# mathjeff/Mapper

Hardware: AMD Instinct MI355X
Metric: M reads/s aligned (150 bp) (higher is better)
Workload: dtype f64

## Files before the change

mapper_amd/csrc/xm_defs.h:

```cpp
#pragma once
#include <stdint.h>
#include <stddef.h>
#include <math.h>
#include <stdlib.h>

#if defined(__HIPCC__)
#include <hip/hip_runtime.h>
#define XM_HD __host__ __device__
#if defined(__HIP_DEVICE_COMPILE__)
#define XM_GLOBAL(T) T __attribute__((address_space(1)))
#define XM_LDS(T) T __attribute__((address_space(3)))
#else
#define XM_GLOBAL(T) T
#define XM_LDS(T) T
#endif
#define XM_INL __host__ __device__ __forceinline__
#ifndef XM_NOINL_LINKAGE
#define XM_NOINL_LINKAGE
#endif
#define XM_NOINL XM_NOINL_LINKAGE __host__ __device__ __noinline__
#define XM_NOINL_DECL XM_NOINL_LINKAGE __host__ __device__
#else
#define XM_HD
#define XM_GLOBAL(T) T
#define XM_LDS(T) T
#define XM_INL inline
#define XM_NOINL
#define XM_NOINL_DECL
#endif

namespace xm {

enum : int32_t {
  XM_OK = 0,
  XM_ST_OVERFLOW = 1,
  XM_ST_OUT_OVERFLOW = 2,
  XM_ST_NEED_GROW = 4,
  XM_ST_INTERNAL = 5,
  XM_ST_NEED_HEAVY = 6,
  XM_ST_NEED_CONF = 11,
};

XM_INL int32_t jadd(int32_t a, int32_t b) { return (int32_t)((uint32_t)a + (uint32_t)b); }
XM_INL int32_t jmul(int32_t a, int32_t b) { return (int32_t)((uint32_t)a * (uint32_t)b); }
XM_INL int32_t jabs(int32_t v) { return v == INT32_MIN ? v : (v < 0 ? -v : v); }
XM_INL int32_t j2i(double d) {
  if (d != d) return 0;
  if (d >= 2147483647.0) return INT32_MAX;
  if (d <= -2147483648.0) return INT32_MIN;
  return (int32_t)d;
}
XM_INL double dmin(double a, double b) { return a < b ? a : b; }
XM_INL double dmax(double a, double b) { return a > b ? a : b; }
XM_INL double jmaxd(double a, double b) {
  if (a != a || b != b) return NAN;
  return a > b ? a : b;
}
XM_INL int imin(int a, int b) { return a < b ? a : b; }
XM_INL int iclamp(int v, int lo, int hi) { return v < lo ? lo : (v > hi ? hi : v); }
XM_INL int imax(int a, int b) { return a > b ? a : b; }
XM_INL int iabs(int a) { return a < 0 ? -a : a; }
XM_INL double jnextUp(double d) {
  if (d != d || d == INFINITY) return d;
  if (d == 0.0) { uint64_t b = 1; double r; __builtin_memcpy(&r, &b, 8); return r; }
  uint64_t b;
  __builtin_memcpy(&b, &d, 8);
  if (d > 0) b += 1; else b -= 1;
  double r;
  __builtin_memcpy(&r, &b, 8);
  return r;
}

XM_INL uint8_t bpComplement(uint8_t b) { return (uint8_t)(((b & 1) << 3) | ((b & 2) << 1) | ((b & 4) >> 1) | ((b & 8) >> 3)); }
XM_INL bool bpCanMatch(uint8_t a, uint8_t b) { return (a & b) != 0; }
XM_INL int bpPop(uint8_t b) { return __builtin_popcount(b & 15); }
XM_INL bool bpIsAmbiguous(uint8_t b) { return bpPop(b) != 1; }
XM_INL bool bpIsFullyAmbiguous(uint8_t b) { return (b & 15) == 15; }
XM_INL double bpFalseNegativeRate(uint8_t b) { int n = bpPop(b); return n <= 1 ? 0.0 : (double)(n - 1) / 3.0; }

struct SeqView {
  const uint8_t* base;
  int32_t len;
  uint8_t rc;
  uint8_t id;
  XM_INL uint8_t at(int i) const { XM_GLOBAL(const uint8_t)* const g = (XM_GLOBAL(const uint8_t)*)base; return rc ? bpComplement(g[len - 1 - i]) : g[i]; }
};

XM_INL uint64_t seqWord8(const SeqView& s, int i) {
  uint64_t x;
  if (!s.rc) {
    __builtin_memcpy(&x, (const void*)(s.base + i), 8);
    return x;
  }
  __builtin_memcpy(&x, (const void*)(s.base + (s.len - 8 - i)), 8);
  x = __builtin_bswap64(x);
  return ((x & 0x0101010101010101ull) << 3) | ((x & 0x0202020202020202ull) << 1) | ((x & 0x0404040404040404ull) >> 1) | ((x & 0x0808080808080808ull) >> 3);
}
XM_INL int seqMatchRun(const SeqView& a, int ai, const SeqView& b, int bi, int limit) {
  int k = 0;
  while (k + 8 <= limit && ai + k + 8 <= a.len && bi + k + 8 <= b.len) {
    const uint64_t t = seqWord8(a, ai + k) & seqWord8(b, bi + k);
    const uint64_t zero = ~(t + 0x7F7F7F7F7F7F7F7Full) & 0x8080808080808080ull;
    if (zero) return k + (__builtin_ctzll(zero) >> 3);
    k += 8;
  }
  while (k < limit && bpCanMatch(a.at(ai + k), b.at(bi + k))) k++;
  return k;
}
XM_INL int seqMatchRunBack(const SeqView& a, int ai, const SeqView& b, int bi, int limit) {
  int k = 0;
  while (k + 8 <= limit && ai - k - 7 >= 0 && bi - k - 7 >= 0) {
    const uint64_t t = seqWord8(a, ai - k - 7) & seqWord8(b, bi - k - 7);
    const uint64_t zero = ~(t + 0x7F7F7F7F7F7F7F7Full) & 0x8080808080808080ull;
    if (zero) return k + (__builtin_clzll(zero) >> 3);
    k += 8;
  }
  while (k < limit && bpCanMatch(a.at(ai - k), b.at(bi - k))) k++;
  return k;
}

XM_INL uint64_t seqAmbiguousBytes(uint64_t x) {
  x &= 0x0F0F0F0F0F0F0F0Full;
  const uint64_t pairs = (x & 0x0505050505050505ull) + ((x >> 1) & 0x0505050505050505ull);
  const uint64_t pop = (pairs & 0x0303030303030303ull) + ((pairs >> 2) & 0x0303030303030303ull);
  const uint64_t bad = pop ^ 0x0101010101010101ull;
  return (bad + 0x7F7F7F7F7F7F7F7Full) & 0x8080808080808080ull;
}
XM_INL uint64_t seqZeroBytes(uint64_t t) { return ~(t + 0x7F7F7F7F7F7F7F7Full) & 0x8080808080808080ull; }
XM_INL int seqCountAmbiguous(const SeqView& s, int start, int end) {
  int n = 0, i = start;
  for (; i + 8 <= end && i + 8 <= s.len && i >= 0; i += 8) n += __builtin_popcountll(seqAmbiguousBytes(seqWord8(s, i)));
  for (; i < end; i++) if (__builtin_popcount(s.at(i) & 15) != 1) n++;
  return n;
}

struct Params {
  double MutationPenalty, InsertionStart_Penalty, InsertionExtension_Penalty, DeletionStart_Penalty, DeletionExtension_Penalty,
      MaxErrorRate, UnalignedPenalty, AmbiguityPenalty, Max_PenaltySpan;
  int32_t MaxNumMatches;
  int32_t StartingInsertionStartFree;
  XM_INL double getStartingInsertionStartPenalty() const { return StartingInsertionStartFree ? 0.0 : InsertionStart_Penalty; }
  XM_INL double getMinPossibleNonzeroPenalty() const {
    double r = MutationPenalty;
    r = dmin(r, getStartingInsertionStartPenalty() + InsertionStart_Penalty);
    r = dmin(r, DeletionStart_Penalty + DeletionExtension_Penalty);
    return r;
  }
  XM_INL double getPenalty(uint8_t q, uint8_t r) const {
    if (!bpCanMatch(r, q)) return MutationPenalty;
    return AmbiguityPenalty * bpFalseNegativeRate((uint8_t)(q | r));
  }
};

struct Table {
  int32_t capacity;
  int32_t maxCount;
  int64_t offBase;
  int64_t posBase;
};
static const uint32_t XM_OVERFULL = 0x80000000u;

struct IndexView {
  int32_t numContigs, minInterestingSize, maxHashedLength, enableGapmers, posIs64;
  int32_t dupWindow;
  double dupGranularity;
  int64_t totalForwardAndReverseSize;
  const int64_t* contigStart;
  const int32_t* contigLen;
  const int64_t* seqCumStart;
  const uint8_t* refCodes;
  const Table* tables;
  const uint32_t* bucketOff;
  const uint32_t* positions32;
  const uint64_t* positions64;
  const int64_t* dupKeyStart;
  const int32_t* dupKeys;
  const uint32_t* lines32;
  const uint64_t* lines64;
  const struct ConfEntry* conf;
  uint32_t confMask;
  struct ConfMiss* confMiss;
  const int32_t* baLogStep;
};
struct ConfEntry { uint64_t penaltyBits; int32_t queryLength; int32_t used; double totalLengthForHighConfidence; };
struct ConfMissKey { uint64_t penaltyBits; int32_t queryLength; int32_t pad; };
struct ConfMiss { unsigned long long n; unsigned long long cap; ConfMissKey keys[1]; };
XM_INL uint32_t confHash(uint64_t penaltyBits, int32_t queryLength) {
  uint64_t x = (penaltyBits ^ (penaltyBits >> 31)) * 0x9E3779B97F4A7C15ull + (uint64_t)(uint32_t)queryLength * 0xC2B2AE3D27D4EB4Full;
  return (uint32_t)(x >> 37);
}
XM_INL bool confLookup(const ConfEntry* table, uint32_t mask, double penalty, int32_t queryLength, double& value) {
  if (!table) return false;
  uint64_t bits;
  __builtin_memcpy(&bits, &penalty, 8);
  uint32_t h = confHash(bits, queryLength) & mask;
  while (true) {
    const ConfEntry e = table[h];
    if (!e.used) return false;
    if (e.penaltyBits == bits && e.queryLength == queryLength) { value = e.totalLengthForHighConfidence; return true; }
    h = (h + 1) & mask;
  }
}
XM_INL int32_t baNumBasesToEncodeReferencePosition(const int32_t* step, int32_t refLen) {
  if (refLen == 0) return INT32_MIN + 1;
  if (refLen < 0) return 1;
  int k = 0;
  while (k + 1 < 24 && refLen >= step[k + 1]) k++;
  return k + 1;
}
constexpr int XM_LINE_SLOTS = 7;
constexpr int64_t XM_LINE_FLAG = 1ll << 62;
template <typename W, typename P>
XM_INL void xmFillLine(W* line, uint32_t o0, uint32_t o1, const P* tablePositions) {
  const uint32_t first = o0 & ~XM_OVERFULL, count = (o1 & ~XM_OVERFULL) - first;
  line[0] = (W)(count | (o0 & XM_OVERFULL));
  for (uint32_t j = 0; j < (uint32_t)XM_LINE_SLOTS; j++) line[1 + j] = ((o0 & XM_OVERFULL) == 0 && j < count) ? (W)tablePositions[first + j] : (W)0;
}

XM_INL SeqView refView(const IndexView& ix, int contig, bool rc) {
  SeqView v;
  v.base = ix.refCodes + ix.contigStart[contig];
  v.len = ix.contigLen[contig];
  v.rc = rc ? 1 : 0;
  v.id = 0;
  return v;
}

struct Caps {
  int32_t scale;
  int32_t heavyAllowed;
  int32_t searchInHbmOnly;
  int32_t maxLevels, maxPyramidBlocks, maxHistory, maxCounters, maxPending, maxQM, maxGoodAlignments, maxBlocks,
      maxNodes, nodeHash, gridCap, maxBuckets, bucketHash, matcherEntries, maxSections, maxPieces, maxCountMap, maxJoined;
};
XM_INL Caps makeCaps(int scale) {
  Caps c;
  c.scale = scale;
  c.heavyAllowed = 2;
  c.searchInHbmOnly = 0;
  c.maxLevels = 48 * scale;
  c.maxPyramidBlocks = 1536 * scale;
  c.maxHistory = 192 * scale;
  c.maxCounters = 96 * scale;
  c.maxPending = 128 * scale;
  c.maxQM = 64 * scale;
  c.maxGoodAlignments = 32 * scale;
  c.maxBlocks = 16 * scale;
  c.maxNodes = 1536 * scale;
  c.nodeHash = 4096 * scale;
// ... 57 lines not shown
```

mapper_amd/csrc/xm_seed.h:

```cpp
#pragma once
#include "xm_defs.h"

#ifndef XM_WALK_INLINE
#define XM_WALK_INLINE 2
#endif
#if XM_WALK_INLINE >= 1
#define XM_NOINL_W1 XM_INL
#else
#define XM_NOINL_W1 XM_NOINL
#endif
#if XM_WALK_INLINE >= 2
#define XM_NOINL_W2 XM_INL
#else
#define XM_NOINL_W2 XM_NOINL
#endif
#if XM_WALK_INLINE == 3
#define XM_NOINL_W3 XM_INL
#else
#define XM_NOINL_W3 XM_NOINL
#endif
#if XM_WALK_INLINE >= 4
#define XM_NOINL_W4 XM_INL
#else
#define XM_NOINL_W4 XM_NOINL
#endif

namespace xm {

struct alignas(16) PBlock {
  uint16_t start, len;
  int32_t fwd, rev;
  uint8_t flags;
  int8_t gapDir;
  int16_t extraGap;
};
enum : uint8_t { F_RML = 1, F_RMR = 2, F_NRML = 4, F_NRMR = 8 };
struct alignas(16) PBlockWord { uint32_t w[4]; };
XM_INL PBlock pbUnpack(const PBlockWord& v) {
  PBlock b;
  b.start = (uint16_t)(v.w[0] & 0xFFFFu); b.len = (uint16_t)(v.w[0] >> 16); b.fwd = (int32_t)v.w[1]; b.rev = (int32_t)v.w[2];
  b.flags = (uint8_t)(v.w[3] & 0xFFu); b.gapDir = (int8_t)((v.w[3] >> 8) & 0xFFu); b.extraGap = (int16_t)(v.w[3] >> 16);
  return b;
}
XM_INL PBlockWord pbPack(const PBlock& b) {
  PBlockWord v;
  v.w[0] = (uint32_t)b.start | ((uint32_t)b.len << 16); v.w[1] = (uint32_t)b.fwd; v.w[2] = (uint32_t)b.rev;
  v.w[3] = (uint32_t)b.flags | ((uint32_t)(uint8_t)b.gapDir << 8) | ((uint32_t)(uint16_t)b.extraGap << 16);
  return v;
}

XM_INL int maxGapmerNumBasepairsUsed(int startingLength) { return startingLength + startingLength * 9 / 8 + 1; }

XM_INL PBlock level0Block(uint8_t code, int index) {
  PBlock b;
  int f = (code == 1) ? 0 : (code == 2) ? 1 : (code == 4) ? 2 : 3;
  b.start = (uint16_t)index;
  b.len = 1;
  b.fwd = f;
  b.rev = 3 - f;
  b.flags = (uint8_t)(((f / 2 == 0) ? F_RML : F_RMR) | ((f % 2 == 0) ? F_NRML : F_NRMR));
  b.gapDir = 0;
  b.extraGap = 0;
  return b;
}

XM_INL int32_t mergeHash(int leftLength, int32_t leftHash, int rightLength, int32_t rightHash) {
  int64_t rotatedLeft = ((int64_t)leftHash + 1) * (54323 + 323 * (int64_t)rightLength);
  int64_t rotatedRight = (int64_t)jadd(rightHash, 1) * (int64_t)leftLength;
  uint64_t top = (uint64_t)rotatedLeft + (uint64_t)rotatedRight;
  return jadd((int32_t)(uint32_t)top, (int32_t)(uint32_t)((uint64_t)((int64_t)top >> 32)));
}

template <typename B>
XM_INL bool shouldMergeBlocks(const B& l, const B& r) {
  if ((int)l.start + l.len < (int)r.start) return false;
  return (l.flags & F_RMR) || (r.flags & F_RML);
}

constexpr uint8_t mergeRule(int anchor, int fr, int aBits, int oBits, int lc) {
  bool rml = true, rmr = true, nrml = true, nrmr = true;
  if (anchor != 0 && fr != 1) {
    bool anchorIsRight = anchor == 2;
    bool isReverse = fr == 0;
    bool invert = isReverse == anchorIsRight;
    bool aL = (aBits & 1) != 0, aR = (aBits & 2) != 0;
    if (aL && aR) { if (anchorIsRight) aR = false; else aL = false; }
    bool oL = (oBits & 1) != 0, oR = (oBits & 2) != 0;
    if (oL && oR) { if (!anchorIsRight) oL = false; else oR = false; }
    rml = aL != invert;
    rmr = aR != invert;
    nrml = oL != invert;
    nrmr = oR != invert;
  }
  if (lc != 1) {
    rml = lc == 2;
    rmr = !rml;
    nrml = !rml;
    nrmr = !nrml;
  }
  if (fr != 1) {
    if (rml && rmr) { rml = fr == 2; rmr = !rml; }
    if (nrml && nrmr) { nrml = rml; nrmr = !nrml; }
  }
  int gd = 0;
  if (rml != rmr) gd = rml ? 1 : -1;
  else if (anchor != 0) gd = (anchor == 2) ? 1 : -1;
  return (uint8_t)((rml ? F_RML : 0) | (rmr ? F_RMR : 0) | (nrml ? F_NRML : 0) | (nrmr ? F_NRMR : 0) | ((gd + 1) << 4));
}
struct MergeRuleTable { uint8_t v[3 * 3 * 4 * 4 * 3]; };
constexpr MergeRuleTable makeMergeRuleTable() {
  MergeRuleTable t{};
  for (int anchor = 0; anchor < 3; anchor++) for (int fr = 0; fr < 3; fr++) for (int a = 0; a < 4; a++) for (int o = 0; o < 4; o++) for (int lc = 0; lc < 3; lc++)
    t.v[(((anchor * 3 + fr) * 4 + a) * 4 + o) * 3 + lc] = mergeRule(anchor, fr, a, o, lc);
  return t;
}
static constexpr MergeRuleTable kMergeRuleHost = makeMergeRuleTable();
#if defined(__HIPCC__)
static __device__ const MergeRuleTable kMergeRuleDev = makeMergeRuleTable();
#endif
#if defined(__HIP_DEVICE_COMPILE__)
__shared__ uint8_t xm_merge_rule_lds[sizeof(MergeRuleTable)];
XM_INL void xmLoadMergeRule() {
  for (int i = (int)threadIdx.x; i < (int)sizeof(MergeRuleTable); i += (int)blockDim.x) xm_merge_rule_lds[i] = kMergeRuleDev.v[i];
  __syncthreads();
}
XM_INL uint8_t mergeRuleLookup(int idx) { return xm_merge_rule_lds[idx]; }
#else
XM_INL void xmLoadMergeRule() {}
XM_INL uint8_t mergeRuleLookup(int idx) { return kMergeRuleHost.v[idx]; }
#endif

template <typename B>
XM_INL B mergeBlocks(const B& L, const B& R) {
  B b;
  int start = L.start, len = (int)R.start + R.len - (int)L.start;
  b.start = (decltype(b.start))start;
  b.len = (decltype(b.len))len;
  b.fwd = mergeHash(L.len, L.fwd, R.len, R.fwd);
  b.rev = mergeHash(R.len, R.rev, L.len, L.rev);
  const int anchor = (L.fwd != R.rev) ? ((L.fwd > R.rev) ? 2 : 1) : 0;
  const int fr = (b.fwd < b.rev) ? 0 : ((b.fwd == b.rev) ? 1 : 2);
  const int lc = (L.len < R.len) ? 0 : ((L.len == R.len) ? 1 : 2);
  const int lBits = (L.flags >> 2) & 3, rBits = (R.flags >> 2) & 3;
  const int aBits = (anchor == 2) ? rBits : lBits, oBits = (anchor == 2) ? lBits : rBits;
  const uint8_t rule = mergeRuleLookup((((anchor * 3 + fr) * 4 + aBits) * 4 + oBits) * 3 + lc);
  b.flags = (uint8_t)(rule & 15);
  b.gapDir = (int8_t)((int)(rule >> 4) - 1);
  b.extraGap = (int16_t)(((int)L.len + (int)R.len - len) / 4);
  return b;
}

struct QBlock {
  int32_t start, len, used, fwd, rev;
  int32_t id;
  uint8_t flags;
  XM_INL int end() const { return start + len; }
  XM_INL bool isPrimaryPolarity() const {
    bool rml = (flags & F_RML) != 0, rmr = (flags & F_RMR) != 0;
    if (rml != rmr) return rml;
    return fwd >= rev;
  }
  XM_INL int32_t lookupKey() const { return isPrimaryPolarity() ? fwd : rev; }
};

XM_INL int gapmerCharCode(uint8_t code) {
  return code == 1 ? 1 : code == 2 ? 2 : code == 4 ? 3 : code == 8 ? 4 : 0;
}

template <typename B>
XM_INL int withGapAndExtension(const B& b, const SeqView& seq, QBlock& out) {
  int targetExtraLength = b.len;
  int32_t mx = b.fwd > b.rev ? b.fwd : b.rev;
  targetExtraLength += jabs(mx) % 3;
  targetExtraLength += b.extraGap;
  int gapLength = b.len / 2;
  int extensionLength = targetExtraLength - gapLength;
  out.flags = 0;
// ... 81 lines not shown
  int32_t* status;
  DevCounters* dc;

  XM_INL void init(const SeqView& s, PBlock* b, int cap_, int32_t* ls, int maxLevels_, int32_t* st) {
    dc = nullptr;
    ms = nullptr;
    seq = s; blocks = b; cap = cap_; levelStart = ls; maxLevels = maxLevels_; nBuilt = 0; used = 0; status = st;
    levelStart[1] = 0;
  }

  XM_INL PBlock entryAt(int level, int i) const {
    if (level > 0) return blocks[levelStart[level] + i];
    uint8_t code = seq.at(i);
    PBlock b = level0Block(code, i);
    if (bpIsAmbiguous(code)) { b.flags = F_MULTI; b.fwd = 0; b.rev = 0; }
    return b;
  }
  XM_INL int numPoss(int level, const PBlock& e) const {
    if (!(e.flags & F_MULTI)) return 1;
    if (level > 0) return e.rev;
    return bpPop(seq.at(e.start));
  }
  XM_INL void possAt(int level, const PBlock& e, int k, PossView& p) const {
    if (!(e.flags & F_MULTI)) { p.block = e; p.cond = &p.own; p.condLen = 0; p.hasBlock = 1; return; }
    if (level > 0) {
      const Poss& s = ms->pool[e.fwd + k];
      p.block = s.block; p.cond = ms->conds + s.condOff; p.condLen = s.condLen; p.hasBlock = s.hasBlock;
      return;
    }
    uint8_t code = seq.at(e.start);
    int seen = 0;
    uint8_t option = 1;
    for (int bit = 0; bit < 4; bit++) {
      uint8_t o = (uint8_t)(1 << bit);
      if (code & o) { if (seen == k) { option = o; break; } seen++; }
    }
    p.block = level0Block(option, e.start);
    p.own = ((CondEnt)e.start << 2) | (CondEnt)(option == 1 ? 0 : option == 2 ? 1 : option == 4 ? 2 : 3);
    p.cond = &p.own; p.condLen = 1;
    p.hasBlock = 1;
  }
  XM_INL bool multiAddOption(int& nOpt, int& nOptCond, const PBlock& block, bool hasBlock, const CondEnt* cond, int condLen) {
    if (ms->poolUsed + nOpt >= ms->poolCap || ms->condUsed + nOptCond + condLen > ms->condCap) return false;
    Poss& o = ms->pool[ms->poolUsed + nOpt];
    o.block = block; o.hasBlock = hasBlock ? 1 : 0; o.pad = 0;
    o.condOff = ms->condUsed + nOptCond; o.condLen = condLen;
    for (int t = 0; t < condLen; t++) ms->conds[o.condOff + t] = cond[t];
    nOpt++; nOptCond += condLen;
    return true;
  }
  XM_INL bool multiExpand(int prev, int n, const PBlock& leftBlock, const CondEnt* leftCond, int leftCondLen, int i, int& nOpt, int& nOptCond) {
    MFrame* const st = ms->frames;
    CondEnt* const sc = ms->stack;
    if (leftCondLen > ms->stackCap || ms->framesCap < 1) return false;
    for (int t = 0; t < leftCondLen; t++) sc[t] = leftCond[t];
    int sp = 0;
    st[0].j = i; st[0].opt = 0; st[0].condOff = 0; st[0].condLen = leftCondLen; st[0].found = 0;
    while (sp >= 0) {
      MFrame& f = st[sp];
      const int nextIdx = f.j + 1;
      if (nextIdx >= n) { sp--; continue; }
      const PBlock next = entryAt(prev, nextIdx);
      if (f.opt >= numPoss(prev, next)) { sp--; continue; }
      PossView ro;
      possAt(prev, next, f.opt, ro);
      f.opt++;
      const int top = f.condOff + f.condLen;
      const int icLen = condIntersect(sc + f.condOff, f.condLen, ro.cond, ro.condLen, sc + top, ms->stackCap - top);
      if (icLen == -2) return false;
      if (icLen < 0) { if (f.found) sp--; continue; }
      f.found = 1;
      if (nOpt > XM_MAX_COMBINATIONS) return true;
      if (!ro.hasBlock) {
        if (sp + 1 >= ms->framesCap) return false;
        sp++;
        st[sp].j = nextIdx; st[sp].opt = 0; st[sp].condOff = top; st[sp].condLen = icLen; st[sp].found = 0;
        continue;
      }
      const bool merge = shouldMergeBlocks(leftBlock, ro.block);
      if (!multiAddOption(nOpt, nOptCond, merge ? mergeBlocks(leftBlock, ro.block) : leftBlock, merge, sc + top, icLen)) return false;
    }
    return true;
  }
  XM_INL void buildLevelMulti() {
    const int prev = nBuilt;
    const int n = count(prev);
    int w = used;
    for (int i = 0; i + 1 < n; i++) {
      const PBlock L = entryAt(prev, i), R = entryAt(prev, i + 1);
      if (!((L.flags | R.flags) & F_MULTI)) {
        if (shouldMergeBlocks(L, R)) {
          if (w >= cap) { *status = XM_ST_OVERFLOW; return; }
          blocks[w++] = mergeBlocks(L, R);
        }
        continue;
      }
      int nOpt = 0, nOptCond = 0;
      const int nl = numPoss(prev, L);
      for (int k = 0; k < nl; k++) {
        PossView lo;
        possAt(prev, L, k, lo);
        if (lo.hasBlock) {
          if (!multiExpand(prev, n, lo.block, lo.cond, lo.condLen, i, nOpt, nOptCond)) { *status = XM_ST_OVERFLOW; return; }
        } else {
          if (!multiAddOption(nOpt, nOptCond, lo.block, false, lo.cond, lo.condLen)) { *status = XM_ST_OVERFLOW; return; }
        }
      }
      if (nOpt > 0 && nOpt <= XM_MAX_COMBINATIONS) {
        int minStart = -1, maxEnd = -1;
        for (int k = 0; k < nOpt; k++) if (ms->pool[ms->poolUsed + k].hasBlock) {
          const PBlock& b = ms->pool[ms->poolUsed + k].block;
          if (minStart < 0 || (int)b.start < minStart) minStart = b.start;
          if ((int)b.start + b.len > maxEnd) maxEnd = (int)b.start + b.len;
        }
        if (minStart >= 0) {
          if (w >= cap) { *status = XM_ST_OVERFLOW; return; }
          PBlock m;
          m.start = (uint16_t)minStart; m.len = (uint16_t)(maxEnd - minStart); m.fwd = ms->poolUsed; m.rev = nOpt; m.flags = F_MULTI; m.gapDir = 0; m.extraGap = 0;
          ms->poolUsed += nOpt; ms->condUsed += nOptCond;
          blocks[w++] = m;
        }
      }
    }
    nBuilt++;
    used = w;
    levelStart[nBuilt + 1] = w;
  }
  XM_INL int count(int level) const { return level == 0 ? seq.len : levelStart[level + 1] - levelStart[level]; }
  XM_INL PBlock blockAt(int level, int i) const { return level == 0 ? level0Block(seq.at(i), i) : blocks[levelStart[level] + i]; }

  XM_NOINL void ensureMulti(int level) {
    while (nBuilt < level) {
      if (nBuilt + 2 >= maxLevels) { *status = XM_ST_OVERFLOW; return; }
      buildLevelMulti();
      if (*status) return;
    }
  }
  XM_NOINL void ensure(int level) {
    if (ms) { ensureMulti(level); return; }
    XM_TIC(t0);
    PBlock* const blk = blocks;
    const int capL = cap;
    const SeqView sq = seq;
    while (nBuilt < level) {
      if (nBuilt + 2 >= maxLevels) { *status = XM_ST_OVERFLOW; return; }
      int prev = nBuilt;
      int n = count(prev);
      int w = used;
      const int base = prev == 0 ? 0 : levelStart[prev];
      bool ovf = false;
      if (n > 1 && prev == 0) {
        XM_GLOBAL(PBlockWord)* const dst = (XM_GLOBAL(PBlockWord)*)blk;
        PBlock L = level0Block(sq.at(0), 0);
        for (int i0 = 0; i0 + 1 < n && !ovf; i0 += 8) {
          uint8_t codes[8];
          const int m = imin(8, n - 1 - i0);
#pragma unroll
          for (int k = 0; k < 8; k++) codes[k] = sq.at(i0 + 1 + (k < m ? k : 0));
#pragma unroll
          for (int k = 0; k < 8; k++) {
            if (k < m && !ovf) {
              const PBlock R = level0Block(codes[k], i0 + 1 + k);
              if (shouldMergeBlocks(L, R)) {
                if (w >= capL) ovf = true;
                else dst[w++] = pbPack(mergeBlocks(L, R));
              }
              L = R;
            }
          }
        }
      } else if (n > 1) {
        XM_GLOBAL(const PBlockWord)* const src = (XM_GLOBAL(const PBlockWord)*)(blk + base);
        XM_GLOBAL(PBlockWord)* const dst = (XM_GLOBAL(PBlockWord)*)blk;
        PBlock L = pbUnpack(src[0]);
        for (int i0 = 0; i0 + 1 < n && !ovf; i0 += 8) {
          PBlockWord buf[8];
          const int m = imin(8, n - 1 - i0);
#pragma unroll
          for (int k = 0; k < 8; k++) buf[k] = src[i0 + 1 + (k < m ? k : 0)];
#pragma unroll
          for (int k = 0; k < 8; k++) {
            if (k < m && !ovf) {
              const PBlock R = pbUnpack(buf[k]);
              if (shouldMergeBlocks(L, R)) {
                if (w >= capL) ovf = true;
                else dst[w++] = pbPack(mergeBlocks(L, R));
              }
              L = R;
            }
          }
        }
      }
      if (ovf) { *status = XM_ST_OVERFLOW; return; }
      nBuilt++;
      used = w;
      levelStart[nBuilt + 1] = w;
    }
    XM_TOC(dc, T_PYRAMID, t0);
  }
  XM_INL bool getAfter(int level, int pos, PBlock& out) {
    if (level == 0) {
      int p = pos + 1;
      if (p >= seq.len) return false;
      out = ms ? entryAt(0, p) : level0Block(seq.at(p), p);
      return true;
    }
    ensure(level);
    if (*status) return false;
    int lo = levelStart[level], hi = levelStart[level + 1];
    while (lo < hi) {
      int mid = (lo + hi) >> 1;
      if ((int)blocks[mid].start > pos) hi = mid; else lo = mid + 1;
    }
    if (lo >= levelStart[level + 1]) return false;
    out = blocks[lo];
    return true;
  }
  XM_INL bool get(int level, int index, PBlock& out) {
    if (level == 0) {
      if (index >= seq.len) return false;
      out = ms ? entryAt(0, index) : level0Block(seq.at(index), index);
      return true;
    }
    if (!getAfter(level, index - 1, out)) return false;
    return (int)out.start == index;
  }
};

XM_INL const Table* containingMap(const IndexView& ix, int used, int32_t* status) {
  if (used > ix.maxHashedLength) { *status = XM_ST_NEED_GROW; return nullptr; }
  return &ix.tables[used];
}
XM_INL uint32_t packedKey(const Table* t, int32_t key) {
  int32_t r = key % t->capacity;
  if (r < 0) r += t->capacity;
  return (uint32_t)r;
}
XM_INL int numMatchesLowerBound(const IndexView& ix, const QBlock& b, DevCounters* dc, int32_t* status) {
  if (b.used < ix.minInterestingSize) return INT32_MAX;
  const Table* t = containingMap(ix, b.used, status);
  if (!t) return INT32_MAX;
  uint32_t k = packedKey(t, b.lookupKey());
  if (dc) dc->headerProbes++;
  if (ix.lines32 || ix.lines64) {
    const uint32_t h = ix.lines64 ? (uint32_t)ix.lines64[(t->offBase + k) * 8] : ix.lines32[(t->offBase + k) * 8];
    return (h & XM_OVERFULL) ? INT32_MAX : (int)h;
  }
  const uint32_t* off = ix.bucketOff + t->offBase + k;
  uint32_t o0 = off[0], o1 = off[1];
  if (o0 & XM_OVERFULL) return INT32_MAX;
  return (int)((o1 & ~XM_OVERFULL) - (o0 & ~XM_OVERFULL));
}
XM_INL int dbMaxNumMatchesAllowed(const IndexView& ix, const QBlock& b, int32_t* status) {
  if (b.used < ix.minInterestingSize) return -1;
  const Table* t = containingMap(ix, b.used, status);
  if (!t) return 0;
  return t->maxCount;
}
struct RefPos { int32_t contig; uint8_t rc; int32_t start; };
XM_INL RefPos decodePosition(const IndexView& ix, int64_t enc) {
  int lo = 0, hi = ix.numContigs * 2;
  while (hi - lo > 1) {
    int mid = (lo + hi) >> 1;
    if (ix.seqCumStart[mid] <= enc) lo = mid; else hi = mid;
  }
  RefPos p;
  p.contig = lo >> 1;
  p.rc = (uint8_t)(lo & 1);
  p.start = (int32_t)(enc - ix.seqCumStart[lo]);
  return p;
}
XM_INL int64_t xmPositionAt(const IndexView& ix, int64_t idx) {
  if (idx & XM_LINE_FLAG) { idx &= ~XM_LINE_FLAG; return ix.lines64 ? (int64_t)ix.lines64[idx] : (int64_t)ix.lines32[idx]; }
  return ix.posIs64 ? (int64_t)ix.positions64[idx] : (int64_t)ix.positions32[idx];
}
XM_INL int matchBlock(const IndexView& ix, const QBlock& b, int64_t& first, bool& invert, DevCounters* dc, int32_t* status) {
  if (b.used < ix.minInterestingSize) return -1;
  const Table* t = containingMap(ix, b.used, status);
  if (!t) return -1;
  uint32_t k = packedKey(t, b.lookupKey());
  if (dc) { dc->headerProbes++; dc->bucketFetches++; }
  int count;
  if (ix.lines32 || ix.lines64) {
    const int64_t line = (t->offBase + k) * 8;
    const uint32_t h = ix.lines64 ? (uint32_t)ix.lines64[line] : ix.lines32[line];
    if (h & XM_OVERFULL) return -1;
    count = (int)h;
    if (count > t->maxCount) return -1;
    if (count <= XM_LINE_SLOTS) first = XM_LINE_FLAG | (line + 1);
    else first = t->posBase + (int64_t)(ix.bucketOff[t->offBase + k] & ~XM_OVERFULL);
  } else {
    const uint32_t* off = ix.bucketOff + t->offBase + k;
    uint32_t o0 = off[0], o1 = off[1];
    if (o0 & XM_OVERFULL) return -1;
    count = (int)((o1 & ~XM_OVERFULL) - (o0 & ~XM_OVERFULL));
    if (count > t->maxCount) return -1;
    first = t->posBase + (int64_t)(o0 & ~XM_OVERFULL);
  }
  invert = !b.isPrimaryPolarity();
  if (dc) dc->hitsFetched += (unsigned long long)count;
  return count;
}
XM_INL RefPos fetchHit(const IndexView& ix, int64_t idx, bool invert, int blockSpan) {
  int64_t enc = xmPositionAt(ix, idx);
  RefPos p = decodePosition(ix, enc);
  if (invert) {
    p.start = ix.contigLen[p.contig] - p.start - blockSpan;
    p.rc ^= 1;
  }
  return p;
}

struct PathState {
  int32_t batchIndex;
  bool curExists;
  PBlock cur;
  bool gapComputed;
  int32_t gapStatus;
  QBlock gap;
  bool havePrev1, havePrev2;
  int32_t prevFwd1, prevFwd2;
};

struct Counter {
  int32_t offset;
  int32_t contig;
  int32_t numMatches, numDistinctMismatches, lastMismatchedPosition, lastMatchedBlockId, historyProcessedIndex, priority;
  int32_t next, prev;
  uint8_t seqAId;
  uint8_t mapSel;
  uint8_t good;
};

struct SeqMatch {
  int32_t offset, contig;
  uint8_t seqAId;
  XM_INL bool reversed() const { return (seqAId & 1) != 0; }
};

struct QMatch {
  int32_t n, priority;
  SeqMatch c[2];
  uint8_t hint;
};

struct ListRef { int32_t id, n; int16_t* items; };

struct ReadCtx;

struct Comp {
  Pyramid pyr;
  PathState path;
  SeqView query, rcQuery;
  Counter* counters; int32_t nCounters;
  int16_t* good; int32_t nGood;
  bool foundGood, done;
  QBlock* history; int32_t nHistory;
  QBlock* pending; int32_t pendHead, pendTail;
  int32_t numBlocksMatchingAnywhere, maxNonoverlappingBlockVisited, numNonoverlappingBlocksVisited, minNumDistinctMismatches;
  int32_t maxIndelLengthToConsider;
  int32_t nextBlockId;
  ListRef hp, best, all;
};

struct SeedEnv {
  const IndexView* ix;
  const Caps* caps;
  DevCounters* dc;
  int32_t* status;
  int32_t* listIdCounter;
  const int32_t* mateLen;
};

XM_INL int seqALen(const SeedEnv& e, uint8_t seqAId) { return e.mateLen[seqAId >> 1]; }
XM_INL int smStartB(const SeqMatch& m) { return imax(0, m.offset); }
XM_INL int smEndB(const SeedEnv& e, const SeqMatch& m) { return imin(m.offset + seqALen(e, m.seqAId), e.ix->contigLen[m.contig]); }
XM_INL bool smEquals(const SeqMatch& a, const SeqMatch& b) { return a.offset == b.offset && a.seqAId == b.seqAId && a.contig == b.contig; }

XM_INL void pathInit(PathState& p) {
  p.batchIndex = -1;
  p.curExists = true;
  p.cur.start = 0; p.cur.len = 0; p.cur.fwd = 0; p.cur.rev = 0; p.cur.flags = 0; p.cur.gapDir = 0; p.cur.extraGap = 0;
  p.gapComputed = false;
  p.gapStatus = 0;
  p.havePrev1 = p.havePrev2 = false;
  p.prevFwd1 = p.prevFwd2 = 0;
}

XM_INL void pathMoveRight(Comp& c) {
  PBlock nb;
  c.path.curExists = c.pyr.getAfter(c.path.batchIndex, c.path.cur.start, nb);
  if (c.path.curExists) c.path.cur = nb;
  c.path.gapComputed = false;
}
XM_INL void pathMoveDown(Comp& c) {
  c.path.batchIndex--;
  PBlock nb;
  c.path.curExists = c.pyr.getAfter(c.path.batchIndex, c.path.cur.start, nb);
  if (c.path.curExists) c.path.cur = nb;
  c.path.gapComputed = false;
}
XM_INL void pathMoveUpOrRight(Comp& c) {
  PBlock up;
  if (c.pyr.get(c.path.batchIndex + 1, c.path.cur.start, up)) {
    c.path.batchIndex++;
    c.path.cur = up;
    c.path.gapComputed = false;
  } else {
    pathMoveRight(c);
  }
}
XM_INL bool pathWithGap(Comp& c, const SeedEnv& e, QBlock& out) {
  if (!e.ix->enableGapmers) {
    const PBlock& b = c.path.cur;
    out.start = b.start; out.len = b.len; out.used = b.len; out.fwd = b.fwd; out.rev = b.rev; out.flags = b.flags; out.id = -1;
    return true;
  }
  if (!c.path.gapComputed) {
    c.path.gapStatus = withGapAndExtension(c.path.cur, c.pyr.seq, c.path.gap);
    c.path.gap.id = -1;
    c.path.gapComputed = true;
  }
  if (c.path.gapStatus == 0) return false;
  out = c.path.gap;
  return true;
}
XM_INL int pathMaxNumMatchesAllowed(Comp& c, const SeedEnv& e, const QBlock& b) {
  if (b.len >= c.query.len / 6) return dbMaxNumMatchesAllowed(*e.ix, b, e.status);
  if (b.flags & F_RMR) return 5;
  return b.used + 1;
}
XM_NOINL_W1 bool pathAdvance(Comp& c, const SeedEnv& e) {
  XM_TIC(t0);
  int singleLen = c.path.cur.len;
  if (maxGapmerNumBasepairsUsed(singleLen) < e.ix->minInterestingSize && e.ix->enableGapmers) {
    pathMoveUpOrRight(c);
  } else {
    QBlock ext;
    if (pathWithGap(c, e, ext)) {
      int numMatches = numMatchesLowerBound(*e.ix, ext, e.dc, e.status);
      if (numMatches < 6) {
        if (c.path.batchIndex > 0) pathMoveDown(c); else pathMoveRight(c);
      } else {
        if (numMatches > pathMaxNumMatchesAllowed(c, e, ext)) pathMoveUpOrRight(c);
        else pathMoveRight(c);
      }
    } else {
      int typical = singleLen * 3 / 2;
      if (typical <= e.ix->minInterestingSize && e.ix->enableGapmers) pathMoveUpOrRight(c);
      else { if (c.path.batchIndex > 0) pathMoveDown(c); else pathMoveRight(c); }
    }
  }
  while (c.path.curExists && (c.path.cur.flags & F_MULTI) && *e.status == 0) {
    if (c.path.batchIndex > 0) pathMoveDown(c); else pathMoveRight(c);
  }
  XM_TOC(e.dc, T_WALK, t0);
  return c.path.curExists && *e.status == 0;
}
XM_NOINL_W1 bool pathNextInterestingBlock(Comp& c, const SeedEnv& e, QBlock& out) {
  if (!c.path.curExists) return false;
  while (true) {
    if (!pathAdvance(c, e)) return false;
    QBlock ext;
    if (!pathWithGap(c, e, ext)) continue;
    int n = numMatchesLowerBound(*e.ix, ext, e.dc, e.status);
    if (*e.status) return false;
    if (!(n <= pathMaxNumMatchesAllowed(c, e, ext))) continue;
    bool seen = false;
    if (c.path.havePrev1 && ext.fwd == c.path.prevFwd1) seen = true;
    else if (c.path.havePrev2 && ext.fwd == c.path.prevFwd2) seen = true;
    c.path.havePrev2 = c.path.havePrev1;
    c.path.prevFwd2 = c.path.prevFwd1;
    c.path.havePrev1 = true;
    c.path.prevFwd1 = ext.fwd;
    if (seen) continue;
    ext.id = c.nextBlockId++;
    out = ext;
    return true;
  }
}

XM_INL void counterUpdate(Comp& c, const SeedEnv& e, Counter& k) {
  while (k.historyProcessedIndex < c.nHistory) {
    const QBlock& b = c.history[k.historyProcessedIndex];
    if (b.id != k.lastMatchedBlockId) {
      if (b.start >= k.lastMismatchedPosition) {
        if (k.offset + b.end() <= e.ix->contigLen[k.contig]) {
          k.numDistinctMismatches++;
          k.lastMismatchedPosition = b.end();
        }
      }
    }
    k.historyProcessedIndex++;
  }
}
XM_INL int counterNumDistinctMismatches(Comp& c, const SeedEnv& e, Counter& k) { counterUpdate(c, e, k); return k.numDistinctMismatches; }
XM_INL void declareGood(Comp& c, const SeedEnv& e, int ci) {
  Counter& k = c.counters[ci];
  if (!k.good) {
    if (c.nGood >= e.caps->maxCounters) { *e.status = XM_ST_OVERFLOW; return; }
    c.good[c.nGood++] = (int16_t)ci;
    k.good = 1;
    k.priority = counterNumDistinctMismatches(c, e, k);
  }
}
XM_INL void compAddMatch(Comp& c, const SeedEnv& e, int ci, const QBlock& qb, int queryBlockNumMatches, const SeqMatch& fullMatch) {
  Counter& k = c.counters[ci];
  k.numMatches++;
  k.lastMatchedBlockId = qb.id;
  counterUpdate(c, e, k);
  if (k.numMatches <= 1) {
    if (k.numMatches == 1) {
      c.foundGood = true;
      declareGood(c, e, ci);
    } else {
      if (queryBlockNumMatches <= qb.len) {
        int distanceFromStart = fullMatch.offset;
        int distanceFromEnd = e.ix->contigLen[fullMatch.contig] - (fullMatch.offset + seqALen(e, fullMatch.seqAId));
        if (imin(distanceFromStart, distanceFromEnd) < 0) declareGood(c, e, ci);
      }
    }
  }
}
XM_NOINL_W3 void compUpdateMatches(Comp& c, const SeedEnv& e, const SeqMatch& m, const QBlock& qb, int queryBlockNumMatches) {
  uint8_t mapSel = m.reversed() ? 0 : 1;
  int cur = -1, lower = -1, higher = -1;
  for (int i = 0; i < c.nCounters; i++) {
    const Counter& k = c.counters[i];
    if (k.mapSel != mapSel || k.contig != m.contig) continue;
    if (k.offset == m.offset) { cur = i; break; }
    if (k.offset < m.offset) { if (lower < 0 || k.offset > c.counters[lower].offset) lower = i; }
    else { if (higher < 0 || k.offset < c.counters[higher].offset) higher = i; }
  }
  if (cur < 0) {
    if (c.nCounters >= e.caps->maxCounters) { *e.status = XM_ST_OVERFLOW; return; }
    cur = c.nCounters++;
    Counter& k = c.counters[cur];
    k.offset = m.offset; k.contig = m.contig; k.seqAId = m.seqAId; k.mapSel = mapSel; k.good = 0;
    k.numMatches = 0;
    k.numDistinctMismatches = c.numNonoverlappingBlocksVisited;
    k.lastMismatchedPosition = qb.start;
    k.lastMatchedBlockId = -2;
    k.historyProcessedIndex = c.nHistory - 1;
    k.priority = 0;
    k.next = k.prev = -1;
    if (lower >= 0 && iabs(c.counters[lower].offset - m.offset) <= c.maxIndelLengthToConsider) {
      k.prev = lower;
      c.counters[lower].next = cur;
    }
    if (higher >= 0 && iabs(c.counters[higher].offset - m.offset) <= c.maxIndelLengthToConsider) {
      k.next = higher;
      c.counters[higher].prev = cur;
    }
  }
  int prev = c.counters[cur].prev;
  if (prev >= 0) compAddMatch(c, e, prev, qb, queryBlockNumMatches, m);
  int next = c.counters[cur].next;
  if (next >= 0) compAddMatch(c, e, next, qb, queryBlockNumMatches, m);
  bool updateThisOne = true;
  if ((prev >= 0 && c.counters[prev].good) || (next >= 0 && c.counters[next].good)) {
    if (!c.counters[cur].good) updateThisOne = false;
  }
  if (updateThisOne) compAddMatch(c, e, cur, qb, queryBlockNumMatches, m);
}

XM_INL int nextCounterInOrder(const Comp& c, uint8_t mapSel, int lastContig, int lastOffset, bool first) {
  int best = -1;
  for (int i = 0; i < c.nCounters; i++) {
    const Counter& k = c.counters[i];
    if (k.mapSel != mapSel) continue;
    if (!first && (k.contig < lastContig || (k.contig == lastContig && k.offset <= lastOffset))) continue;
    if (best < 0 || k.contig < c.counters[best].contig || (k.contig == c.counters[best].contig && k.offset < c.counters[best].offset)) best = i;
  }
  return best;
}
XM_NOINL_W2 void tryEnsureGoodMatchCounter(Comp& c, const SeedEnv& e) {
  if (!c.foundGood && c.nCounters <= c.query.len) {
    for (int mapSel = 0; mapSel < 2; mapSel++) {
      int lc = 0, lo = 0;
      bool first = true;
      while (true) {
        int i = nextCounterInOrder(c, (uint8_t)mapSel, lc, lo, first);
        if (i < 0) break;
        first = false; lc = c.counters[i].contig; lo = c.counters[i].offset;
        declareGood(c, e, i);
      }
    }
    c.foundGood = true;
  }
}

XM_NOINL_W2 bool compNextInterestingBlock(Comp& c, const SeedEnv& e, QBlock& out) {
  c.all.id = 0;
  while (true) {
    QBlock b;
    if (!pathNextInterestingBlock(c, e, b)) {
      if (*e.status) return false;
      if (c.pendHead >= c.pendTail) return false;
      out = c.pending[c.pendHead++];
      return true;
    }
    if (b.start < c.maxNonoverlappingBlockVisited) {
      if (c.pendTail >= e.caps->maxPending) { *e.status = XM_ST_OVERFLOW; return false; }
      c.pending[c.pendTail++] = b;
      continue;
    }
    out = b;
    return true;
  }
}

XM_NOINL_W4 bool compStep(Comp& c, const SeedEnv& e) {
  if (c.done) return false;
  QBlock qb;
  int64_t first = 0;
  bool invert = false;
  int nHits;
  while (true) {
    if (!compNextInterestingBlock(c, e, qb)) {
      if (*e.status) return false;
      c.done = true;
      if (c.numBlocksMatchingAnywhere < 1) tryEnsureGoodMatchCounter(c, e);
      return false;
    }
    nHits = matchBlock(*e.ix, qb, first, invert, e.dc, e.status);
    if (*e.status) return false;
    if (nHits < 0) continue;
    break;
  }
  if (c.nHistory >= e.caps->maxHistory) { *e.status = XM_ST_OVERFLOW; return false; }
  c.history[c.nHistory++] = qb;
  const IndexView& ix = *e.ix;
  XM_TIC(tHits);
  for (int h = 0; h < nHits; h++) {
    RefPos rp = fetchHit(ix, first + h, invert, qb.len);
    SeqView refSeq = refView(ix, rp.contig, rp.rc != 0);
    int numMismatchedItems = 0, numMatchedItems = 0;
    for (int distance = 1; distance < 20; distance++) {
      int checkOffset = -distance;
      int queryIndex = qb.start + checkOffset;
      if (queryIndex >= 0 && queryIndex < c.query.len) {
        int referenceIndex = rp.start + checkOffset;
        if (referenceIndex >= 0 && referenceIndex < refSeq.len) {
          if (!bpCanMatch(c.query.at(queryIndex), refSeq.at(referenceIndex))) numMismatchedItems++; else numMatchedItems++;
        }
      }
      checkOffset = qb.len - 1 + distance;
      queryIndex = qb.start + checkOffset;
      if (queryIndex >= 0 && queryIndex < c.query.len) {
        int referenceIndex = rp.start + checkOffset;
        if (referenceIndex >= 0 && referenceIndex < refSeq.len) {
          if (!bpCanMatch(c.query.at(queryIndex), refSeq.at(referenceIndex))) numMismatchedItems++; else numMatchedItems++;
        }
      }
      if (numMatchedItems < numMismatchedItems) break;
      if (numMatchedItems >= numMismatchedItems + qb.used) break;
    }
    if (numMismatchedItems > numMatchedItems) continue;
    SeqMatch fm;
    fm.contig = rp.contig;
    if (rp.rc) {
      int reverseQueryBlockStart = c.query.len - qb.end();
      int reverseReferenceBlockStart = refSeq.len - (rp.start + qb.len);
      fm.offset = reverseReferenceBlockStart - reverseQueryBlockStart;
      fm.seqAId = c.rcQuery.id;
    } else {
      fm.offset = rp.start - qb.start;
      fm.seqAId = c.query.id;
    }
    compUpdateMatches(c, e, fm, qb, nHits);
    if (*e.status) return false;
  }
  XM_TOC(e.dc, T_HITS, tHits);
  if (qb.start >= c.maxNonoverlappingBlockVisited) {
    c.maxNonoverlappingBlockVisited = qb.end();
    c.numNonoverlappingBlocksVisited++;
  }
  c.numBlocksMatchingAnywhere++;
  c.minNumDistinctMismatches = -1;
  return true;
}

XM_NOINL ListRef compFindGoodPositionsHavingPriorityUpTo(Comp& c, const SeedEnv& e, int priority) {
  while (true) {
    if (c.numNonoverlappingBlocksVisited >= jadd(priority, 1)) break;
    if (!compStep(c, e)) break;
  }
  if (c.hp.id != 0 && c.hp.n == c.nGood) return c.hp;
  int n = 0;
  for (int i = 0; i < c.nGood; i++) {
    if (c.counters[c.good[i]].priority <= priority) c.hp.items[n++] = c.good[i];
  }
  c.hp.n = n;
  c.hp.id = ++(*e.listIdCounter);
  return c.hp;
}
XM_NOINL ListRef compGetAllPositions(Comp& c, const SeedEnv& e) {
  if (c.all.id == 0) {
    int n = 0;
    for (int mapSel = 0; mapSel < 2; mapSel++) {
      int lc = 0, lo = 0;
      bool first = true;
      while (true) {
        int i = nextCounterInOrder(c, (uint8_t)mapSel, lc, lo, first);
        if (i < 0) break;
        first = false; lc = c.counters[i].contig; lo = c.counters[i].offset;
        c.all.items[n++] = (int16_t)i;
      }
    }
    c.all.n = n;
    c.all.id = ++(*e.listIdCounter);
  }
  return c.all;
}
XM_NOINL ListRef compGetBestMatches(Comp& c, const SeedEnv& e) {
  c.best.id = ++(*e.listIdCounter);
  c.best.n = 0;
  if (c.numBlocksMatchingAnywhere < 1) return c.best;
  if (c.minNumDistinctMismatches < 0) {
    int mn = c.numNonoverlappingBlocksVisited - 1;
    for (int i = 0; i < c.nGood; i++) {
      int cnt = counterNumDistinctMismatches(c, e, c.counters[c.good[i]]);
      if (mn >= cnt) mn = cnt;
    }
    c.minNumDistinctMismatches = mn;
  }
  int mn = c.minNumDistinctMismatches;
  int n = 0;
  for (int i = 0; i < c.nGood; i++) {
    int cnt = counterNumDistinctMismatches(c, e, c.counters[c.good[i]]);
    if (cnt <= mn) c.best.items[n++] = c.good[i];
  }
  c.best.n = n;
  return c.best;
}

struct PathsCounter {
  Comp* comps;
  int32_t nComps;
  int32_t maxOffsetBetweenComponents;
  bool foundNonemptyResult;
  bool havePrevious;
  int32_t prevListId[2];
  QMatch* assembled; int32_t nAssembled;
  QMatch* filtered; int32_t nFiltered;
  int16_t* nearby;
};

XM_INL SeqMatch counterMatch(const Counter& k) { SeqMatch m; m.offset = k.offset; m.contig = k.contig; m.seqAId = k.seqAId; return m; }

XM_INL int countPriority(const PathsCounter& pc, const SeedEnv& e, int c0, int c1) {
  const Counter& a = pc.comps[0].counters[c0];
  const Counter& b = pc.comps[1].counters[c1];
  SeqMatch m1 = counterMatch(a), m2 = counterMatch(b);
  if (smStartB(m1) < smEndB(e, m2) && smEndB(e, m1) > smStartB(m2)) return imax(imax(0, a.priority), b.priority);
  return a.priority + b.priority;
}

XM_NOINL void pcMatchWithoutCache(PathsCounter& pc, const SeedEnv& e, const ListRef* lists) {
  pc.nAssembled = 0;
  if (pc.nComps == 1) {
    for (int i = 0; i < lists[0].n; i++) {
      if (pc.nAssembled >= e.caps->maxQM) { *e.status = XM_ST_OVERFLOW; return; }
      const Counter& k = pc.comps[0].counters[lists[0].items[i]];
      QMatch& q = pc.assembled[pc.nAssembled++];
      q.n = 1; q.priority = k.priority; q.c[0] = counterMatch(k); q.hint = 0;
    }
    return;
  }
  bool lastComponentIsLargest = lists[0].n <= lists[1].n;
  int firstComp = lastComponentIsLargest ? 0 : 1;
  int secondComp = 1 - firstComp;
  Comp& FC = pc.comps[firstComp];
  Comp& SC = pc.comps[secondComp];
  for (int j = 0; j < lists[secondComp].n; j++) {
    int ci = lists[secondComp].items[j];
    const Counter& k = SC.counters[ci];
    int querySequenceLength = seqALen(e, k.seqAId);
    int maxReverseOffset = querySequenceLength / 2;
    bool sequenceMatchReversed = (k.seqAId & 1) != 0;
    bool queryMatchReversed = (sequenceMatchReversed == (secondComp % 2 == 0));
    int offset = k.offset;
    int searchStart, searchEnd;
    bool otherSequenceExpectEarlier = (queryMatchReversed == lastComponentIsLargest);
    if (otherSequenceExpectEarlier) { searchStart = offset - maxReverseOffset; searchEnd = jadd(offset, pc.maxOffsetBetweenComponents); }
    else { searchStart = offset - pc.maxOffsetBetweenComponents; searchEnd = offset + maxReverseOffset; }
    if (searchStart > searchEnd) { *e.status = XM_ST_INTERNAL; return; }
    int nn = 0;
    for (int i = 0; i < lists[firstComp].n; i++) {
      int fi = lists[firstComp].items[i];
      const Counter& f = FC.counters[fi];
      bool fRev = (f.seqAId & 1) != 0;
      bool fQueryMatchReversed = (fRev == (firstComp % 2 == 0));
      if (fQueryMatchReversed != queryMatchReversed || f.contig != k.contig) continue;
      if (f.offset < searchStart || f.offset > searchEnd) continue;
      int p = nn++;
      while (p > 0 && FC.counters[pc.nearby[p - 1]].offset > f.offset) { pc.nearby[p] = pc.nearby[p - 1]; p--; }
      pc.nearby[p] = (int16_t)fi;
    }
    bool descending = queryMatchReversed && nn > 1;
    for (int t = 0; t < nn; t++) {
      int fi = pc.nearby[descending ? nn - 1 - t : t];
      int c0 = lastComponentIsLargest ? fi : ci;
      int c1 = lastComponentIsLargest ? ci : fi;
      if (pc.nAssembled >= e.caps->maxQM) { *e.status = XM_ST_OVERFLOW; return; }
      QMatch& q = pc.assembled[pc.nAssembled++];
      q.n = 2;
      q.c[0] = counterMatch(pc.comps[0].counters[c0]);
      q.c[1] = counterMatch(pc.comps[1].counters[c1]);
      q.hint = counterNumDistinctMismatches(pc.comps[0], e, pc.comps[0].counters[c0]) < counterNumDistinctMismatches(pc.comps[1], e, pc.comps[1].counters[c1]) ? 1 : 0;
// ... 93 lines not shown
```

Before: 15.78.

## Use index hints for pyramid walk, word-wide flank checks and level-1 loads

Tracks the current block index along the pyramid walk so moving right becomes a direct next-element load, and moving up or down uses an interpolated guess plus galloping search instead of a full binary search. Flank mismatch counting around each seed hit now reads 8-base words and builds match bitmasks instead of comparing one base at a time. Level-1 pyramid construction reads eight bases in one word. It also adds optional host-side counters and a correctness cross-check. The aim is fewer scattered global loads in the seed stage, in exchange for more register state and extra branching.

```diff
diff --git a/mapper_amd/csrc/xm_defs.h b/mapper_amd/csrc/xm_defs.h
--- a/mapper_amd/csrc/xm_defs.h
+++ b/mapper_amd/csrc/xm_defs.h
@@ -95,6 +95,23 @@
   __builtin_memcpy(&x, (const void*)(s.base + (s.len - 8 - i)), 8);
   x = __builtin_bswap64(x);
   return ((x & 0x0101010101010101ull) << 3) | ((x & 0x0202020202020202ull) << 1) | ((x & 0x0404040404040404ull) >> 1) | ((x & 0x0808080808080808ull) >> 3);
+}
+XM_INL uint64_t seqWindow8(const SeqView& s, int i) {
+  if (s.len >= 8) {
+    const int j = iclamp(i, 0, s.len - 8);
+    const uint64_t w = seqWord8(s, j);
+    const int k = i - j;
+    if (k == 0) return w;
+    if (k >= 8 || k <= -8) return 0;
+    return k > 0 ? w >> (8 * k) : w << (-8 * k);
+  }
+  uint64_t w = 0;
+  for (int k = 0; k < 8; k++) { const int p = i + k; if (p >= 0 && p < s.len) w |= (uint64_t)s.at(p) << (8 * k); }
+  return w;
+}
+XM_INL uint32_t seqNonzeroBits(uint64_t t) {
+  const uint64_t nz = (((t & 0x7F7F7F7F7F7F7F7Full) + 0x7F7F7F7F7F7F7F7Full) | t) & 0x8080808080808080ull;
+  return (uint32_t)(((nz >> 7) * 0x0102040810204080ull) >> 56);
 }
 XM_INL int seqMatchRun(const SeqView& a, int ai, const SeqView& b, int bi, int limit) {
   int k = 0;
diff --git a/mapper_amd/csrc/xm_seed.h b/mapper_amd/csrc/xm_seed.h
--- a/mapper_amd/csrc/xm_seed.h
+++ b/mapper_amd/csrc/xm_seed.h
@@ -23,6 +23,35 @@
 #define XM_NOINL_W4 XM_INL
 #else
 #define XM_NOINL_W4 XM_NOINL
+#endif
+
+#ifndef XM_WALK_HINT
+#define XM_WALK_HINT 1
+#endif
+#ifndef XM_FLANK_WORDS
+#define XM_FLANK_WORDS 1
+#endif
+#ifndef XM_LEVEL1_WORDS
+#define XM_LEVEL1_WORDS 1
+#endif
+#if defined(XM_WALK_COUNT) && !defined(__HIPCC__)
+namespace xm {
+struct WalkCounts { unsigned long long getAfterCalls, getAfterLoads, flankLoads, flankHits, level1Loads, moveRight, moveDown, moveUpOrRight; };
+inline WalkCounts xmWalkCounts;
+inline bool xmWalkCountOn = false;
+}
+#define XM_WC(field, n) do { if (xm::xmWalkCountOn) xm::xmWalkCounts.field += (unsigned long long)(n); } while (0)
+#else
+#define XM_WC(field, n) do { } while (0)
+#endif
+#if defined(XM_WALK_CHECK) && !defined(__HIPCC__)
+namespace xm {
+struct WalkCheck { unsigned long long lookups, failures; };
+inline WalkCheck xmWalkCheck;
+}
+#define XM_WALK_CHECKED 1
+#else
+#define XM_WALK_CHECKED 0
 #endif
 
 namespace xm {
@@ -410,11 +439,20 @@
       if (n > 1 && prev == 0) {
         XM_GLOBAL(PBlockWord)* const dst = (XM_GLOBAL(PBlockWord)*)blk;
         PBlock L = level0Block(sq.at(0), 0);
+        XM_WC(level1Loads, 1);
         for (int i0 = 0; i0 + 1 < n && !ovf; i0 += 8) {
           uint8_t codes[8];
           const int m = imin(8, n - 1 - i0);
+#if XM_LEVEL1_WORDS
+          const uint64_t word = seqWindow8(sq, i0 + 1);
+          XM_WC(level1Loads, 1);
+#pragma unroll
+          for (int k = 0; k < 8; k++) codes[k] = (uint8_t)(word >> (8 * k));
+#else
+          XM_WC(level1Loads, 8);
 #pragma unroll
           for (int k = 0; k < 8; k++) codes[k] = sq.at(i0 + 1 + (k < m ? k : 0));
+#endif
 #pragma unroll
           for (int k = 0; k < 8; k++) {
             if (k < m && !ovf) {
@@ -465,15 +503,78 @@
     }
     ensure(level);
     if (*status) return false;
+    XM_WC(getAfterCalls, 1);
     int lo = levelStart[level], hi = levelStart[level + 1];
     while (lo < hi) {
       int mid = (lo + hi) >> 1;
+      XM_WC(getAfterLoads, 1);
       if ((int)blocks[mid].start > pos) hi = mid; else lo = mid + 1;
     }
     if (lo >= levelStart[level + 1]) return false;
+    XM_WC(getAfterLoads, 1);
     out = blocks[lo];
     return true;
   }
+#if XM_WALK_HINT
+  XM_INL PBlock blockWord(int at) const { return pbUnpack(((XM_GLOBAL(const PBlockWord)*)blocks)[at]); }
+  XM_INL bool getNext(int level, int at, PBlock& out) {
+    if (*status) return false;
+    XM_WC(getAfterCalls, 1);
+    XM_WC(getAfterLoads, 1);
+    const int end = levelStart[level + 1];
+    const PBlock b = blockWord(imin(at + 1, cap - 1));
+    if (at + 1 >= end) return false;
+    out = b;
+    return true;
+  }
+  XM_INL bool getAfterFrom(int level, int pos, int lo, int hi, int i, int fromCount, int bias, PBlock& out, int& idx) {
+    if (nBuilt < level) ensure(level);
+    if (*status) return false;
+    XM_WC(getAfterCalls, 1);
+    const int first = levelStart[level], n = levelStart[level + 1] - first;
+    if (hi > n) hi = n;
+    PBlock top = PBlock();
+    bool haveTop = false;
+    if (lo < hi) {
+      const int g = iclamp((int)((float)i * (float)n / (float)fromCount) + bias, lo, hi - 1);
+      const PBlock bg = blockWord(first + g), bp = blockWord(first + (g > lo ? g - 1 : g));
+      XM_WC(getAfterLoads, 1);
+      if ((int)bg.start > pos) {
+        hi = g; top = bg; haveTop = true;
+        if (g > lo) {
+          if ((int)bp.start > pos) {
+            hi = g - 1; top = bp;
+            for (int step = 2; hi - step >= lo; step *= 2) {
+              const PBlock b = blockWord(first + hi - step);
+              XM_WC(getAfterLoads, 1);
+              if ((int)b.start > pos) { hi -= step; top = b; } else { lo = hi - step + 1; break; }
+            }
+          } else lo = g;
+        }
+      } else {
+        lo = g + 1;
+        for (int step = 1; lo + step - 1 < hi; step *= 2) {
+          const int p = lo + step - 1;
+          const PBlock b = blockWord(first + p);
+          XM_WC(getAfterLoads, 1);
+          if ((int)b.start > pos) { hi = p; top = b; haveTop = true; break; }
+          lo = p + 1;
+        }
+      }
+      while (lo < hi) {
+        const int mid = (lo + hi) >> 1;
+        const PBlock b = blockWord(first + mid);
+        XM_WC(getAfterLoads, 1);
+        if ((int)b.start > pos) { hi = mid; top = b; haveTop = true; } else lo = mid + 1;
+      }
+    }
+    idx = hi;
+    if (hi >= n) return false;
+    if (!haveTop) { top = blockWord(first + hi); XM_WC(getAfterLoads, 1); }
+    out = top;
+    return true;
+  }
+#endif
   XM_INL bool get(int level, int index, PBlock& out) {
     if (level == 0) {
       if (index >= seq.len) return false;
@@ -578,6 +679,7 @@
   QBlock gap;
   bool havePrev1, havePrev2;
   int32_t prevFwd1, prevFwd2;
+  int32_t curIdx, curAt;
 };
 
 struct Counter {
@@ -643,27 +745,85 @@
   p.gapStatus = 0;
   p.havePrev1 = p.havePrev2 = false;
   p.prevFwd1 = p.prevFwd2 = 0;
-}
-
+  p.curIdx = -1; p.curAt = 0;
+}
+
+#if XM_WALK_HINT
+XM_INL void pathCheckLookup(Comp& c, int level, int pos, bool found, const PBlock& b) {
+#if XM_WALK_CHECKED
+  PBlock want;
+  const bool wantFound = c.pyr.getAfter(level, pos, want);
+  xmWalkCheck.lookups++;
+  if (wantFound != found || (found && (want.start != b.start || want.len != b.len || want.fwd != b.fwd || want.rev != b.rev || want.flags != b.flags ||
+                                       want.gapDir != b.gapDir || want.extraGap != b.extraGap))) xmWalkCheck.failures++;
+#endif
+}
+XM_INL bool pathHasIndex(const Comp& c) { return c.path.batchIndex >= 1 && c.path.curIdx >= 0 && !c.pyr.ms; }
+#endif
 XM_INL void pathMoveRight(Comp& c) {
+  XM_WC(moveRight, 1);
   PBlock nb;
+#if XM_WALK_HINT
+  if (pathHasIndex(c)) {
+    c.path.curExists = c.pyr.getNext(c.path.batchIndex, c.path.curAt, nb);
+    pathCheckLookup(c, c.path.batchIndex, c.path.cur.start, c.path.curExists, nb);
+    if (c.path.curExists) { c.path.cur = nb; c.path.curIdx++; c.path.curAt++; }
+    c.path.gapComputed = false;
+    return;
+  }
+  c.path.curIdx = -1;
+#endif
   c.path.curExists = c.pyr.getAfter(c.path.batchIndex, c.path.cur.start, nb);
   if (c.path.curExists) c.path.cur = nb;
   c.path.gapComputed = false;
 }
 XM_INL void pathMoveDown(Comp& c) {
+  XM_WC(moveDown, 1);
+  PBlock nb;
+#if XM_WALK_HINT
+  if (pathHasIndex(c) && c.path.batchIndex >= 2) {
+    const int level = --c.path.batchIndex, i = c.path.curIdx;
+    int idx;
+    c.path.curExists = c.pyr.getAfterFrom(level, c.path.cur.start, i + 1, INT32_MAX, i, c.pyr.count(level + 1), 1, nb, idx);
+    pathCheckLookup(c, level, c.path.cur.start, c.path.curExists, nb);
+    if (c.path.curExists) { c.path.cur = nb; c.path.curIdx = idx; c.path.curAt = c.pyr.levelStart[level] + idx; }
+    c.path.gapComputed = false;
+    return;
+  }
+  c.path.curIdx = -1;
+#endif
   c.path.batchIndex--;
-  PBlock nb;
   c.path.curExists = c.pyr.getAfter(c.path.batchIndex, c.path.cur.start, nb);
   if (c.path.curExists) c.path.cur = nb;
   c.path.gapComputed = false;
 }
 XM_INL void pathMoveUpOrRight(Comp& c) {
+  XM_WC(moveUpOrRight, 1);
   PBlock up;
+#if XM_WALK_HINT
+  if (!c.pyr.ms && (c.path.batchIndex == 0 || pathHasIndex(c))) {
+    const int level = c.path.batchIndex + 1, i = c.path.batchIndex == 0 ? (int)c.path.cur.start : c.path.curIdx;
+    int idx;
+    const bool found = c.pyr.getAfterFrom(level, (int)c.path.cur.start - 1, 0, i, i, c.pyr.count(level - 1), 0, up, idx);
+    pathCheckLookup(c, level, (int)c.path.cur.start - 1, found, up);
+    if (found && up.start == c.path.cur.start) {
+      c.path.batchIndex++;
+      c.path.cur = up;
+      c.path.curIdx = idx; c.path.curAt = c.pyr.levelStart[level] + idx;
+      c.path.gapComputed = false;
+    } else {
+      pathMoveRight(c);
+    }
+    return;
+  }
+#endif
   if (c.pyr.get(c.path.batchIndex + 1, c.path.cur.start, up)) {
     c.path.batchIndex++;
     c.path.cur = up;
     c.path.gapComputed = false;
+#if XM_WALK_HINT
+    c.path.curIdx = -1;
+#endif
   } else {
     pathMoveRight(c);
   }
@@ -868,6 +1028,16 @@
   }
 }
 
+XM_INL uint32_t distanceBits(int lo, int hi) {
+  lo = imax(lo, 1); hi = imin(hi, 19);
+  return hi < lo ? 0u : (((1u << hi) - 1u) & ~((1u << (lo - 1)) - 1u));
+}
+XM_INL void flankWords(const SeqView& query, const SeqView& ref, int qStart, int rStart, int qEnd, int rEnd, int j, uint32_t& canL, uint32_t& canR) {
+  const uint64_t l = seqWindow8(query, qStart - 8 * (j + 1)) & seqWindow8(ref, rStart - 8 * (j + 1));
+  const uint64_t r = seqWindow8(query, qEnd + 8 * j) & seqWindow8(ref, rEnd + 8 * j);
+  canL |= seqNonzeroBits(__builtin_bswap64(l)) << (8 * j);
+  canR |= seqNonzeroBits(r) << (8 * j);
+}
 XM_NOINL_W4 bool compStep(Comp& c, const SeedEnv& e) {
   if (c.done) return false;
   QBlock qb;
@@ -894,12 +1064,34 @@
     RefPos rp = fetchHit(ix, first + h, invert, qb.len);
     SeqView refSeq = refView(ix, rp.contig, rp.rc != 0);
     int numMismatchedItems = 0, numMatchedItems = 0;
+    XM_WC(flankHits, 1);
+#if XM_FLANK_WORDS
+    const int qEnd = qb.start + qb.len, rEnd = rp.start + qb.len;
+    uint32_t canL = 0, canR = 0;
+    flankWords(c.query, refSeq, qb.start, rp.start, qEnd, rEnd, 0, canL, canR);
+    XM_WC(flankLoads, 4);
+    const uint32_t inL = distanceBits(imax(qb.start - c.query.len + 1, rp.start - refSeq.len + 1), imin(qb.start, rp.start));
+    const uint32_t inR = distanceBits(imax(1 - qEnd, 1 - rEnd), imin(c.query.len - qEnd, refSeq.len - rEnd));
+    for (int distance = 1; distance < 20; distance++) {
+      if (distance == 9) {
+        flankWords(c.query, refSeq, qb.start, rp.start, qEnd, rEnd, 1, canL, canR);
+        flankWords(c.query, refSeq, qb.start, rp.start, qEnd, rEnd, 2, canL, canR);
+        XM_WC(flankLoads, 8);
+      }
+      const uint32_t bit = 1u << (distance - 1);
+      if (inL & bit) { if (!(canL & bit)) numMismatchedItems++; else numMatchedItems++; }
+      if (inR & bit) { if (!(canR & bit)) numMismatchedItems++; else numMatchedItems++; }
+      if (numMatchedItems < numMismatchedItems) break;
+      if (numMatchedItems >= numMismatchedItems + qb.used) break;
+    }
+#else
     for (int distance = 1; distance < 20; distance++) {
       int checkOffset = -distance;
       int queryIndex = qb.start + checkOffset;
       if (queryIndex >= 0 && queryIndex < c.query.len) {
         int referenceIndex = rp.start + checkOffset;
         if (referenceIndex >= 0 && referenceIndex < refSeq.len) {
+          XM_WC(flankLoads, 2);
           if (!bpCanMatch(c.query.at(queryIndex), refSeq.at(referenceIndex))) numMismatchedItems++; else numMatchedItems++;
         }
       }
@@ -908,12 +1100,14 @@
       if (queryIndex >= 0 && queryIndex < c.query.len) {
         int referenceIndex = rp.start + checkOffset;
         if (referenceIndex >= 0 && referenceIndex < refSeq.len) {
+          XM_WC(flankLoads, 2);
           if (!bpCanMatch(c.query.at(queryIndex), refSeq.at(referenceIndex))) numMismatchedItems++; else numMatchedItems++;
         }
       }
       if (numMatchedItems < numMismatchedItems) break;
       if (numMatchedItems >= numMismatchedItems + qb.used) break;
     }
+#endif
     if (numMismatchedItems > numMatchedItems) continue;
     SeqMatch fm;
     fm.contig = rp.contig;
```

Measured after the change: 13.43. 0.851x the previous value.
